# Murmeldyret/cubesat-APDS

Measured on AMD Instinct MI355X. Metric: frames/sec (detect+match+homography) 4k×4k tile vs 1M-desc DB; Mmatches/sec, higher is better.
Workload: dtype fp4 e2m1 operands / f32 accumulate = exact integer Hamming (match), f32 (AKAZE), f64 (homography solve)

## Files before the change

### cubesat-apds_amd/csrc/hamming_mfma.hip

```cpp
#include <atomic>
#include <memory>

#include "config.h"
#include "kernels.h"

namespace apds {

typedef int hm_v8i __attribute__((ext_vector_type(8)));
typedef float hm_f32x4 __attribute__((ext_vector_type(4)));
typedef uint32_t hm_u32x4 __attribute__((ext_vector_type(4)));

#ifndef APDS_HM_WAVES
#define APDS_HM_WAVES 8
#endif
static constexpr int HM_WAVES = APDS_HM_WAVES;
static constexpr int HM_TM = 16 * HM_WAVES;
#ifndef APDS_HM_WPE
#define APDS_HM_WPE 4
#endif
#ifndef APDS_HM_NC
#define APDS_HM_NC 3
#endif
static constexpr int HM_NC = APDS_HM_NC;
static constexpr int HM_Q = HM_WAVES * 16 * HM_NC;
static constexpr int HM_UNIT_SCALE = 0x7F7F7F7F;
static constexpr uint64_t HM_EMPTY = ~0ull;
static constexpr int HM_BIAS = 1024;

__device__ __forceinline__ uint32_t hm_spread8(uint32_t b, uint32_t nib) {
    uint32_t t = b & 0xFFu;
    t = (t | (t << 12)) & 0x000F000Fu;
    t = (t | (t << 6)) & 0x03030303u;
    t = (t | (t << 3)) & 0x11111111u;
    return t * nib;
}

__global__ __launch_bounds__(256) void hm_expand_rows_kernel(const uint32_t* __restrict__ rows, long long n, uint32_t nib, int bias, uint4* __restrict__ out,
                                                             float* __restrict__ pc) {
    APDS_RAISE_WAVE_PRIORITY();
    const long long i = (long long)blockIdx.x * 256 + threadIdx.x;
    const uint32_t d = i < n * 16 ? rows[i] : 0u;
    int v = __popc(d);
#pragma unroll
    for (int off = 8; off > 0; off >>= 1) v += __shfl_xor(v, off);
    if (i >= n * 16) return;
    out[i] = make_uint4(hm_spread8(d, nib), hm_spread8(d >> 8, nib), hm_spread8(d >> 16, nib), hm_spread8(d >> 24, nib));
    if ((threadIdx.x & 15) == 0) pc[i >> 4] = (float)(v + bias);
}

__global__ void hm_pad_rows_kernel(uint4* __restrict__ rows, float* __restrict__ pc, long long n, long long n_pad) {
    const long long i = n + (threadIdx.x >> 4);
    if (i >= n_pad) return;
    for (long long r = i; r < n_pad; r += 8) {
        rows[r * 16 + (threadIdx.x & 15)] = make_uint4(0, 0, 0, 0);
        if ((threadIdx.x & 15) == 0) pc[r] = INFINITY;
    }
}

__global__ void hm_thresholds_kernel(const uint64_t* __restrict__ topk, int K, const float* __restrict__ qpc, int nq, uint32_t* __restrict__ thr) {
    const int i = blockIdx.x * blockDim.x + threadIdx.x;
    if (i >= nq) return;
    const uint64_t k2 = topk[(size_t)i * K + K - 1];
    thr[i] = k2 == HM_EMPTY ? 0x7F800000u : __float_as_uint((float)((int)(uint32_t)(k2 >> 32) - (int)qpc[i] + HM_BIAS));
}

struct HmTop2 {
    uint32_t d0, d1;
    uint32_t i0, i1;
};
__device__ __forceinline__ void hm_insert(HmTop2& b, uint32_t d, uint32_t idx) {
    if (d < b.d1) {
        if (d < b.d0) {
            b.d1 = b.d0;
            b.i1 = b.i0;
            b.d0 = d;
            b.i0 = idx;
        } else {
            b.d1 = d;
            b.i1 = idx;
        }
    }
}

__device__ __forceinline__ void hm_dma_rows(const unsigned char* tile_base, const int (&voff)[4], uint32_t lds_dst) {
    uint32_t keep;
    asm volatile(
        "s_mov_b32 %0, m0\n\t"
        "s_mov_b32 m0, %6\n\t"
        "s_nop 0\n\t"
        "global_load_lds_dwordx4 %1, %5\n\t"
        "global_load_lds_dwordx4 %2, %5 offset:1024\n\t"
        "global_load_lds_dwordx4 %3, %5 offset:2048\n\t"
        "global_load_lds_dwordx4 %4, %5 offset:3072\n\t"
        "s_mov_b32 m0, %0"
        : "=&s"(keep)
        : "v"(voff[0]), "v"(voff[1]), "v"(voff[2]), "v"(voff[3]), "s"(tile_base), "s"(lds_dst)
        : "memory");
}
__device__ __forceinline__ void hm_dma_popcounts(const float* src, int voff, uint32_t lds_dst) {
    uint32_t keep;
    asm volatile(
        "s_mov_b32 %0, m0\n\t"
        "s_mov_b32 m0, %3\n\t"
        "s_nop 0\n\t"
        "global_load_lds_dword %1, %2\n\t"
        "s_mov_b32 m0, %0"
        : "=&s"(keep)
        : "v"(voff), "s"(src), "s"(lds_dst)
        : "memory");
}
__device__ __forceinline__ void hm_dma_wait() { asm volatile("s_waitcnt vmcnt(0)" ::: "memory"); }
template <class T>
__device__ __forceinline__ void hm_settle(T& v) { asm volatile("" : "+v"(v)); }

template <int NC, int PRIO, class Rank>
__device__ __forceinline__ void hm_scan_tiles(const uint4* __restrict__ train_fp4, const float* __restrict__ tpc, int tile_begin, int tile_end,
                                              uint4 (&B)[NC][4], uint32_t index_base, Rank&& rank) {
    extern __shared__ __attribute__((aligned(128))) unsigned char hm_lds[];
    constexpr int TILE_BYTES = HM_TM * 256;
    const int lane = threadIdx.x & 63, wave = __builtin_amdgcn_readfirstlane(threadIdx.x >> 6);
    const int col = lane & 15, kq = lane >> 4;
    const uint32_t lds0 = (uint32_t)(__SIZE_TYPE__)(__attribute__((address_space(3))) unsigned char*)hm_lds;
    int voff[4];
#pragma unroll
    for (int i = 0; i < 4; i++) {
        const int r = 16 * wave + 4 * i + (lane >> 4);
        voff[i] = r * 256 + (((lane & 15) ^ (r & 15)) << 4) - 1024 * i;
    }
    auto stage = [&](int tile, int buf) {
        hm_dma_rows(reinterpret_cast<const unsigned char*>(train_fp4) + (size_t)tile * TILE_BYTES, voff, lds0 + buf * TILE_BYTES + 16 * wave * 256);
        if (wave < HM_TM / 64) hm_dma_popcounts(tpc + (size_t)tile * HM_TM + 64 * wave, 4 * lane, lds0 + 2 * TILE_BYTES + buf * (HM_TM * 4) + 256 * wave);
    };
    typedef const __attribute__((address_space(3))) hm_u32x4* lds_u4;
    typedef const __attribute__((address_space(3))) hm_f32x4* lds_f4;
    uint32_t ra[4], rn = lds0 + 2 * TILE_BYTES + 16 * kq;
#pragma unroll
    for (int s = 0; s < 4; s++) ra[s] = lds0 + col * 256 + (((4 * s + kq) ^ col) << 4);

    hm_u32x4 a[4];
    hm_f32x4 init;
    auto read_block = [&](int rb) {
#pragma unroll
        for (int s = 0; s < 4; s++) a[s] = *(lds_u4)(__SIZE_TYPE__)(ra[s] + rb * 4096);
        init = *(lds_f4)(__SIZE_TYPE__)(rn + rb * 64);
    };

#pragma unroll
    for (int c = 0; c < NC; c++)
#pragma unroll
        for (int s = 0; s < 4; s++) hm_settle(B[c][s].x), hm_settle(B[c][s].y), hm_settle(B[c][s].z), hm_settle(B[c][s].w);
    hm_dma_wait();
    stage(tile_begin, 0);
    hm_dma_wait();
    __syncthreads();
    read_block(0);
    hm_f32x4 acc[NC];
    for (int tile = tile_begin; tile < tile_end; tile++) {
        const int buf = (tile - tile_begin) & 1;
        if (tile + 1 < tile_end) stage(tile + 1, buf ^ 1);
#pragma unroll
        for (int rb = 0; rb < HM_TM / 16; rb++) {
            if (PRIO) __builtin_amdgcn_s_setprio(PRIO);
#pragma unroll
            for (int s = 0; s < 4; s++) {
                const hm_v8i A = {(int)a[s].x, (int)a[s].y, (int)a[s].z, (int)a[s].w, 0, 0, 0, 0};
#pragma unroll
                for (int c = 0; c < NC; c++) {
                    const hm_v8i Bv = {(int)B[c][s].x, (int)B[c][s].y, (int)B[c][s].z, (int)B[c][s].w, 0, 0, 0, 0};
                    acc[c] = __builtin_amdgcn_mfma_scale_f32_16x16x128_f8f6f4(A, Bv, s == 0 ? init : acc[c], 4, 4, 0, HM_UNIT_SCALE, 0, HM_UNIT_SCALE);
                }
            }
            if (PRIO) __builtin_amdgcn_s_setprio(0);
            if (rb + 1 < HM_TM / 16) {
                read_block(rb + 1);
            } else {
                hm_dma_wait();
                __syncthreads();
#pragma unroll
                for (int s = 0; s < 4; s++) ra[s] += buf ? -TILE_BYTES : TILE_BYTES;
                rn += buf ? -HM_TM * 4 : HM_TM * 4;
                read_block(0);
            }
#pragma unroll
            for (int c = 0; c < NC; c++) hm_settle(acc[c]);
            __builtin_amdgcn_sched_barrier(0);
            rank(acc, (uint32_t)(tile * HM_TM + rb * 16 + 4 * kq) + index_base);
        }
    }
}

template <int PRIO, bool THR>
__global__ __launch_bounds__(64 * HM_WAVES) __attribute__((amdgpu_waves_per_eu(APDS_HM_WPE, APDS_HM_WPE))) void hamming_mfma_kernel(const uint4* __restrict__ train_fp4, const float* __restrict__ tpc, int n_train,
                                                           const uint4* __restrict__ query_fp4, const float* __restrict__ qpc, int nq, int tiles_per_split,
                                                           int q_tiles, int splits, uint32_t index_base, const uint32_t* __restrict__ thr,
                                                           uint64_t* __restrict__ out) {
    const int tid = threadIdx.x, lane = tid & 63, wave = tid >> 6;
    int split, qtile;
    if ((splits & 7) == 0) {
        const int xcd = blockIdx.x & 7, j = blockIdx.x >> 3;
        split = xcd + 8 * (j / q_tiles);
        qtile = j % q_tiles;
    } else {
        split = blockIdx.x / q_tiles;
        qtile = blockIdx.x % q_tiles;
    }
    const int q0 = qtile * HM_Q + wave * 16 * HM_NC;
    const int n_tiles = (n_train + HM_TM - 1) / HM_TM;
    const int tile_begin = split * tiles_per_split, tile_end = min(n_tiles, tile_begin + tiles_per_split);
    const int col = lane & 15, kq = lane >> 4;

    uint4 B[HM_NC][4];
    float qq[HM_NC];
#pragma unroll
    for (int c = 0; c < HM_NC; c++) {
        const int qi = min(q0 + 16 * c + col, nq - 1);
#pragma unroll
        for (int s = 0; s < 4; s++) B[c][s] = query_fp4[(size_t)qi * 16 + 4 * s + kq];
        qq[c] = qpc[qi];
    }
    HmTop2 best[HM_NC];
#pragma unroll
    for (int c = 0; c < HM_NC; c++) {
        best[c].d0 = THR ? thr[min(q0 + 16 * c + col, nq - 1)] : 0x7F800000u;
        hm_settle(best[c].d0), hm_settle(qq[c]);
        best[c].d1 = best[c].d0;
        best[c].i0 = best[c].i1 = 0xFFFFFFFFu;
    }

    if (tile_begin < tile_end) {
        hm_scan_tiles<HM_NC, PRIO>(train_fp4, tpc, tile_begin, tile_end, B, index_base, [&](const hm_f32x4 (&a)[HM_NC], uint32_t row0) {
            bool hit[HM_NC];
#pragma unroll
            for (int c = 0; c < HM_NC; c++) {
                const uint32_t mn = min(min(__float_as_uint(a[c][0]), __float_as_uint(a[c][1])), min(__float_as_uint(a[c][2]), __float_as_uint(a[c][3])));
                hit[c] = mn < best[c].d1;
            }
#pragma unroll
            for (int c = 0; c < HM_NC; c++)
                if (__any(hit[c])) {
#pragma unroll
                    for (int j = 0; j < 4; j++) hm_insert(best[c], __float_as_uint(a[c][j]), row0 + j);
                }
        });
    }
#pragma unroll
    for (int c = 0; c < HM_NC; c++) {
        HmTop2 b = best[c];
#pragma unroll
        for (int off = 16; off < 64; off <<= 1) {
            const uint32_t od0 = (uint32_t)__shfl_xor((int)b.d0, off), od1 = (uint32_t)__shfl_xor((int)b.d1, off);
            const uint32_t oi0 = (uint32_t)__shfl_xor((int)b.i0, off), oi1 = (uint32_t)__shfl_xor((int)b.i1, off);
            HmTop2 m = b;
            auto ins = [&](uint32_t d, uint32_t i) {
                if (i == 0xFFFFFFFFu) return;
                if (d < m.d0 || (d == m.d0 && i < m.i0)) {
                    m.d1 = m.d0;
                    m.i1 = m.i0;
                    m.d0 = d;
                    m.i0 = i;
                } else if ((d < m.d1 || (d == m.d1 && i < m.i1)) && i != m.i0) {
                    m.d1 = d;
                    m.i1 = i;
                }
            };
            ins(od0, oi0);
            ins(od1, oi1);
            b = m;
        }
        const int qi = q0 + 16 * c + col;
        if (kq == 0 && qi < nq) {
            uint64_t* o = out + ((size_t)split * nq + qi) * 2;
            o[0] = b.i0 == 0xFFFFFFFFu ? HM_EMPTY : ((uint64_t)(uint32_t)((int)(qq[c] + __uint_as_float(b.d0)) - HM_BIAS) << 32) | b.i0;
            o[1] = b.i1 == 0xFFFFFFFFu ? HM_EMPTY : ((uint64_t)(uint32_t)((int)(qq[c] + __uint_as_float(b.d1)) - HM_BIAS) << 32) | b.i1;
        }
    }
}

template <int K>
struct HmTopK {
    uint32_t d[K];
    uint32_t i[K];
};
template <int K>
__device__ __forceinline__ void hm_insert_k(HmTopK<K>& b, uint32_t d, uint32_t idx) {
#pragma unroll
    for (int j = K - 1; j > 0; j--) {
        const bool shift = d < b.d[j - 1], here = d < b.d[j];
        b.i[j] = shift ? b.i[j - 1] : (here ? idx : b.i[j]);
        b.d[j] = shift ? b.d[j - 1] : (here ? d : b.d[j]);
    }
    const bool first = d < b.d[0];
    b.i[0] = first ? idx : b.i[0];
    b.d[0] = first ? d : b.d[0];
}
__device__ __forceinline__ uint64_t hm_shfl_xor_u64(uint64_t v, int off) {
    return ((uint64_t)(uint32_t)__shfl_xor((int)(uint32_t)(v >> 32), off) << 32) | (uint32_t)__shfl_xor((int)(uint32_t)v, off);
}

#ifndef APDS_HM_NC_K4
#define APDS_HM_NC_K4 2
#endif
#ifndef APDS_HM_NC_K8
#define APDS_HM_NC_K8 2
#endif
template <int K>
struct HmShape {
    static constexpr int NC = K <= 4 ? APDS_HM_NC_K4 : APDS_HM_NC_K8;
    static constexpr int Q = HM_WAVES * 16 * NC;
};

template <int K, int NC, int PRIO, bool THR>
__global__ __launch_bounds__(64 * HM_WAVES) __attribute__((amdgpu_waves_per_eu(APDS_HM_WPE, APDS_HM_WPE))) void hamming_mfma_topk_kernel(
    const uint4* __restrict__ train_fp4, const float* __restrict__ tpc, int n_train, const uint4* __restrict__ query_fp4, const float* __restrict__ qpc, int nq,
    int tiles_per_split, int q_tiles, int splits, uint32_t index_base, const uint32_t* __restrict__ thr, uint64_t* __restrict__ out) {
    const int tid = threadIdx.x, lane = tid & 63, wave = tid >> 6;
    int split, qtile;
    if ((splits & 7) == 0) {
        const int xcd = blockIdx.x & 7, j = blockIdx.x >> 3;
        split = xcd + 8 * (j / q_tiles);
        qtile = j % q_tiles;
    } else {
        split = blockIdx.x / q_tiles;
        qtile = blockIdx.x % q_tiles;
    }
    const int q0 = qtile * (HM_WAVES * 16 * NC) + wave * 16 * NC;
    const int n_tiles = (n_train + HM_TM - 1) / HM_TM;
    const int tile_begin = split * tiles_per_split, tile_end = min(n_tiles, tile_begin + tiles_per_split);
    const int col = lane & 15, kq = lane >> 4;

    uint4 B[NC][4];
    float qq[NC];
#pragma unroll
    for (int c = 0; c < NC; c++) {
        const int qi = min(q0 + 16 * c + col, nq - 1);
#pragma unroll
        for (int s = 0; s < 4; s++) B[c][s] = query_fp4[(size_t)qi * 16 + 4 * s + kq];
        qq[c] = qpc[qi];
    }
    HmTopK<K> best[NC];
#pragma unroll
    for (int c = 0; c < NC; c++) {
        uint32_t start = THR ? thr[min(q0 + 16 * c + col, nq - 1)] : 0x7F800000u;
        hm_settle(start), hm_settle(qq[c]);
#pragma unroll
        for (int j = 0; j < K; j++) best[c].d[j] = start, best[c].i[j] = 0xFFFFFFFFu;
    }

    if (tile_begin < tile_end) {
        hm_scan_tiles<NC, PRIO>(train_fp4, tpc, tile_begin, tile_end, B, index_base, [&](const hm_f32x4 (&a)[NC], uint32_t row0) {
            bool hit[NC];
#pragma unroll
            for (int c = 0; c < NC; c++) {
                const uint32_t mn = min(min(__float_as_uint(a[c][0]), __float_as_uint(a[c][1])), min(__float_as_uint(a[c][2]), __float_as_uint(a[c][3])));
                hit[c] = mn < best[c].d[K - 1];
            }
#pragma unroll
            for (int c = 0; c < NC; c++)
                if (__any(hit[c])) {
#pragma unroll
                    for (int j = 0; j < 4; j++) {
                        const uint32_t v = __float_as_uint(a[c][j]);
                        if (__any(v < best[c].d[K - 1])) hm_insert_k<K>(best[c], v, row0 + j);
                    }
                }
        });
    }
#pragma unroll
    for (int c = 0; c < NC; c++) {
        uint64_t key[K];
#pragma unroll
        for (int j = 0; j < K; j++) key[j] = ((uint64_t)best[c].d[j] << 32) | best[c].i[j];
#pragma unroll
        for (int off = 16; off < 64; off <<= 1) {
            uint64_t other[K];
#pragma unroll
            for (int j = 0; j < K; j++) other[j] = hm_shfl_xor_u64(key[j], off);
#pragma unroll
            for (int j = 0; j < K; j++) key[j] = min(key[j], other[K - 1 - j]);
#pragma unroll
            for (int step = K / 2; step > 0; step >>= 1)
#pragma unroll
                for (int j = 0; j < K; j++)
                    if ((j & step) == 0) {
                        const uint64_t lo = min(key[j], key[j + step]), hi = max(key[j], key[j + step]);
                        key[j] = lo;
                        key[j + step] = hi;
                    }
        }
        const int qi = q0 + 16 * c + col;
        if (kq == 0 && qi < nq) {
            uint64_t* o = out + ((size_t)split * nq + qi) * K;
#pragma unroll
            for (int j = 0; j < K; j++) {
                const uint32_t d = (uint32_t)(key[j] >> 32), i = (uint32_t)key[j];
                o[j] = i == 0xFFFFFFFFu ? HM_EMPTY : ((uint64_t)(uint32_t)((int)(qq[c] + __uint_as_float(d)) - HM_BIAS) << 32) | i;
            }
        }
    }
}

static int hm_list_len(int k) { return k <= 2 ? 2 : (k <= 4 ? 4 : 8); }
static int hm_queries_per_block(int K) { return K <= 2 ? HM_Q : (K <= 4 ? HmShape<4>::Q : HmShape<8>::Q); }

HmPlan hm_plan(int nq, long long nt, int K) {
    HmPlan p;
    p.q_tiles = ceil_div(nq, hm_queries_per_block(K));
    const int t_tiles = (int)ceil_div(nt, (long long)HM_TM);
    constexpr int SLOTS = 256 * (16 / HM_WAVES);
    constexpr int OVERHEAD = 4;
    const int max_splits = (int)std::max<long long>(1, std::min<long long>(std::min(t_tiles, 128), (32ll << 20) / std::max(K, 2) / std::max(nq, 1)));
    long long best_cost = -1;
    p.splits = 1;
    for (int sp = 1; sp <= max_splits; sp++) {
        const long long rounds = ceil_div((long long)p.q_tiles * sp, (long long)SLOTS);
        const long long cost = rounds * (ceil_div(t_tiles, sp) + OVERHEAD);
        if (best_cost < 0 || cost < best_cost) best_cost = cost, p.splits = sp;
    }
    if (config().match_mfma_xcd && t_tiles >= 64) {
        long long best8 = -1;
        int sp8 = 0;
        for (int sp = 8; sp <= std::min(max_splits, 32); sp += 8) {
            const long long rounds = ceil_div((long long)p.q_tiles * sp, (long long)SLOTS);
            const long long cost = rounds * (ceil_div(t_tiles, sp) + OVERHEAD);
            if (best8 < 0 || cost < best8) best8 = cost, sp8 = sp;
        }
        if (sp8 && best8 * 100 <= best_cost * 105) {
            p.splits = sp8;
            p.tiles_per_split = ceil_div(t_tiles, p.splits);
            return p;
        }
    }
    if (config().match_mfma_splits > 0) p.splits = std::min(t_tiles, config().match_mfma_splits);
    p.tiles_per_split = ceil_div(t_tiles, p.splits);
    p.splits = ceil_div(t_tiles, p.tiles_per_split);
    return p;
}

void hm_expand_device(const void* rows64, long long n, bool query, void* out_fp4, float* pc, hipStream_t s) {
    if (n <= 0) return;
    hipLaunchKernelGGL(hm_expand_rows_kernel, dim3((unsigned)ceil_div(n * 16, 256)), dim3(256), 0, s, static_cast<const uint32_t*>(rows64), n, query ? 0xCu : 0x2u,
                       query ? 0 : HM_BIAS, static_cast<uint4*>(out_fp4), pc);
    if (!query && hm_padded_rows(n) > n)
        hipLaunchKernelGGL(hm_pad_rows_kernel, dim3(1), dim3(128), 0, s, static_cast<uint4*>(out_fp4), pc, n, hm_padded_rows(n));
}
long long hm_padded_rows(long long n) { return ceil_div(n, (long long)HM_TM) * HM_TM; }
long long hm_sample_rows(long long nt) {
    const long long cap = config().match_mfma_sample;
    return (cap > 0 && nt >= 65536) ? std::min<long long>(cap, nt / 16 / HM_TM * HM_TM) / HM_TM * HM_TM : 0;
}

template <int K>
static void hm_scan_k_launch(const void* q_fp4, const float* qpc, int nq, const void* t_fp4, const float* tpc, long long nt, const HmPlan& p, uint32_t index_base,
                             uint64_t* parts, hipStream_t s, const uint32_t* thr, size_t lds) {
    constexpr int NC = HmShape<K>::NC;
    static std::atomic<bool> opted_dev[64];
    std::atomic<bool>& opted = opted_dev[ctx().device & 63];
    if (!opted.load()) {
        auto opt = [&](auto kernel) { HIP_CHECK(hipFuncSetAttribute(reinterpret_cast<const void*>(kernel), hipFuncAttributeMaxDynamicSharedMemorySize, 160 * 1024)); };
        opt(&hamming_mfma_topk_kernel<K, NC, 0, false>), opt(&hamming_mfma_topk_kernel<K, NC, 2, false>);
        opt(&hamming_mfma_topk_kernel<K, NC, 0, true>), opt(&hamming_mfma_topk_kernel<K, NC, 2, true>);
        opted.store(true);
    }
    auto go = [&](auto kernel) {
        hipLaunchKernelGGL(kernel, dim3((unsigned)p.q_tiles * p.splits), dim3(64 * HM_WAVES), lds, s, static_cast<const uint4*>(t_fp4), tpc, (int)nt,
                           static_cast<const uint4*>(q_fp4), qpc, nq, p.tiles_per_split, p.q_tiles, p.splits, index_base, thr, parts);
    };
    const bool prio = config().match_mfma_prio > 0;
    if (thr) prio ? go(&hamming_mfma_topk_kernel<K, NC, 2, true>) : go(&hamming_mfma_topk_kernel<K, NC, 0, true>);
    else prio ? go(&hamming_mfma_topk_kernel<K, NC, 2, false>) : go(&hamming_mfma_topk_kernel<K, NC, 0, false>);
}

void hm_scan_device(const void* q_fp4, const float* qpc, int nq, const void* t_fp4, const float* tpc, long long nt, const HmPlan& p, uint32_t index_base,
                    uint64_t* parts, hipStream_t s, const uint32_t* thr, bool timed, int K) {
    const size_t lds = (size_t)2 * HM_TM * 256 + 2 * HM_TM * sizeof(float) + (size_t)std::max(0, config().match_mfma_lds_pad);
    if (K > 2) {
        APDS_REQUIRE(K == 4 || K == 8, APDS_ERR_ASSERT, "the matrix-core matcher keeps lists of 2, 4 or 8");
        std::unique_ptr<KernelTimer> timer, timer_k;
        if (timed) timer.reset(new KernelTimer("hamming_topk", s)), timer_k.reset(new KernelTimer("hamming_topk_mfma_k", s));
        if (K == 4) hm_scan_k_launch<4>(q_fp4, qpc, nq, t_fp4, tpc, nt, p, index_base, parts, s, thr, lds);
        else hm_scan_k_launch<8>(q_fp4, qpc, nq, t_fp4, tpc, nt, p, index_base, parts, s, thr, lds);
        return;
    }
    static std::atomic<bool> opted_dev[64];
    std::atomic<bool>& opted = opted_dev[ctx().device & 63];
    if (!opted.load()) {
        auto opt = [&](auto kernel) { HIP_CHECK(hipFuncSetAttribute(reinterpret_cast<const void*>(kernel), hipFuncAttributeMaxDynamicSharedMemorySize, 160 * 1024)); };
        opt(&hamming_mfma_kernel<0, false>), opt(&hamming_mfma_kernel<1, false>), opt(&hamming_mfma_kernel<2, false>), opt(&hamming_mfma_kernel<3, false>);
        opt(&hamming_mfma_kernel<0, true>), opt(&hamming_mfma_kernel<1, true>), opt(&hamming_mfma_kernel<2, true>), opt(&hamming_mfma_kernel<3, true>);
        opted.store(true);
    }
    std::unique_ptr<KernelTimer> timer;
    if (timed) timer.reset(new KernelTimer("hamming_topk", s));
    auto go = [&](auto kernel) {
        hipLaunchKernelGGL(kernel, dim3((unsigned)p.q_tiles * p.splits), dim3(64 * HM_WAVES), lds, s, static_cast<const uint4*>(t_fp4), tpc, (int)nt,
                           static_cast<const uint4*>(q_fp4), qpc, nq, p.tiles_per_split, p.q_tiles, p.splits, index_base, thr, parts);
    };
    const int prio = std::max(0, std::min(3, config().match_mfma_prio));
    if (thr) {
        switch (prio) {
            case 0: go(&hamming_mfma_kernel<0, true>); break;
            case 1: go(&hamming_mfma_kernel<1, true>); break;
            case 2: go(&hamming_mfma_kernel<2, true>); break;
            default: go(&hamming_mfma_kernel<3, true>); break;
        }
    } else {
        switch (prio) {
            case 0: go(&hamming_mfma_kernel<0, false>); break;
            case 1: go(&hamming_mfma_kernel<1, false>); break;
            case 2: go(&hamming_mfma_kernel<2, false>); break;
            default: go(&hamming_mfma_kernel<3, false>); break;
        }
    }
}

void* hm_train_create(const void* rows64, long long n, hipStream_t s) {
    APDS_REQUIRE(rows64 && n > 0 && n < (1ll << 31), APDS_ERR_ASSERT, "an expanded train set needs rows");
    HmTrain* t = new HmTrain();
    t->device = ctx().device;
    t->src = rows64;
    t->n = n;
    if (hipMalloc(&t->rows, (size_t)hm_padded_rows(n) * 256) != hipSuccess || hipMalloc(reinterpret_cast<void**>(&t->pc), (size_t)hm_padded_rows(n) * 4) != hipSuccess) {
        (void)hipGetLastError();
        if (t->rows) (void)hipFree(t->rows);
        delete t;
        fail(APDS_ERR_NOMEM, "no device memory for the expanded train rows");
    }
    hm_expand_device(rows64, n, false, t->rows, t->pc, s);
    HIP_CHECK(hipStreamSynchronize(s));
    return t;
}
void hm_train_destroy(void* h) {
    HmTrain* t = static_cast<HmTrain*>(h);
    if (!t) return;
    int previous = -1;
    if (hipGetDevice(&previous) != hipSuccess) previous = -1;
    (void)hipSetDevice(t->device);
    (void)hipDeviceSynchronize();
    if (t->rows) (void)hipFree(t->rows);
    if (t->pc) (void)hipFree(t->pc);
    delete t;
    if (previous >= 0) (void)hipSetDevice(previous);
}

static void hm_topk_expanded(const void* q, int nq, const void* t4, const float* tp, long long nt, uint32_t index_base, int k, uint64_t* out, hipStream_t s) {
    ThreadCtx& c = ctx();
    void* q4 = c.alloc((size_t)nq * 256);
    float* qp = c.alloc_n<float>(nq);
    {
        KernelTimer timer("hamming_topk_sample", s);
        hm_expand_device(q, nq, true, q4, qp, s);
    }
    const long long sample = hm_sample_rows(nt);
    const int K = hm_list_len(k);
    uint64_t* topk = k == K ? out : c.alloc_n<uint64_t>((size_t)nq * K);
    if (sample) {
        const HmPlan pa = hm_plan(nq, sample, K), pb = hm_plan(nq, nt - sample, K);
        uint64_t* parts_a = c.alloc_n<uint64_t>((size_t)pa.splits * nq * K);
        uint64_t* parts_b = c.alloc_n<uint64_t>((size_t)(pb.splits + 1) * nq * K);
        uint64_t* topk_a = parts_b + (size_t)pb.splits * nq * K;
        uint32_t* thr = c.alloc_n<uint32_t>(nq);
        {
            KernelTimer timer("hamming_topk_sample", s);
            hm_scan_device(q4, qp, nq, t4, tp, sample, pa, index_base, parts_a, s, nullptr, false, K);
            if (pa.splits > 1) merge_topk_device(parts_a, pa.splits, nq, K, topk_a, s);
            else HIP_CHECK(hipMemcpyAsync(topk_a, parts_a, (size_t)nq * K * 8, hipMemcpyDeviceToDevice, s));
            hipLaunchKernelGGL(hm_thresholds_kernel, dim3(ceil_div(nq, 256)), dim3(256), 0, s, (const uint64_t*)topk_a, K, (const float*)qp, nq, thr);
        }
        hm_scan_device(q4, qp, nq, static_cast<const char*>(t4) + (size_t)sample * 256, tp + sample, nt - sample, pb, index_base + (uint32_t)sample, parts_b, s, thr,
                       true, K);
        merge_topk_device(parts_b, pb.splits + 1, nq, K, topk, s);
    } else {
        const HmPlan p = hm_plan(nq, nt, K);
        uint64_t* parts = p.splits == 1 ? topk : c.alloc_n<uint64_t>((size_t)p.splits * nq * K);
        hm_scan_device(q4, qp, nq, t4, tp, nt, p, index_base, parts, s, nullptr, true, K);
        if (p.splits > 1) merge_topk_device(parts, p.splits, nq, K, topk, s);
    }
    if (k != K) take_first_columns_device(topk, nq, K, k, out, s);
    HIP_CHECK(hipGetLastError());
}

void hamming_mfma_topk_device(const void* q, int nq, const void* t, long long nt, uint32_t index_base, int k, uint64_t* out, hipStream_t s) {
    APDS_REQUIRE(k >= 1 && k <= 8, APDS_ERR_ASSERT, "the matrix-core matcher serves 1 <= k <= 8");
    APDS_REQUIRE(nq > 0 && nt > 0 && nt < (1ll << 31), APDS_ERR_ASSERT, "the matrix-core matcher needs queries and train rows");
    ThreadCtx& c = ctx();
    void* t4 = c.alloc((size_t)hm_padded_rows(nt) * 256);
    float* tp = c.alloc_n<float>(hm_padded_rows(nt));
    {
        KernelTimer timer("hamming_topk_sample", s);
        hm_expand_device(t, nt, false, t4, tp, s);
    }
    hm_topk_expanded(q, nq, t4, tp, nt, index_base, k, out, s);
}

void hamming_mfma_topk_train_device(const void* q, int nq, const void* train, uint32_t index_base, int k, uint64_t* out, hipStream_t s) {
    const HmTrain* t = static_cast<const HmTrain*>(train);
    APDS_REQUIRE(t && k >= 1 && k <= 8 && nq > 0, APDS_ERR_ASSERT, "the matrix-core matcher needs an expanded train set, queries and 1 <= k <= 8");
    hm_topk_expanded(q, nq, t->rows, t->pc, t->n, index_base, k, out, s);
}

}
```

Baseline: 149.7.

## Software-pipeline MFMA Hamming scan with inline asm interleaving previous block's rank test

Replaces the compiler-scheduled MFMA loop with hand-written inline-asm blocks. The min/compare filter for the previous row block is interleaved between the MFMAs of the current one, using two ping-pong accumulator sets, and a drain step handles the final block. The aim is to hide the rank-test VALU work and the MFMA result latency behind matrix-core issue instead of serialising them. It also defers the query popcount load to the epilogue to free registers. This adds fragile asm with hard-coded operand modifiers and an s_nop hazard, supports only NC of 2 or 3, and increases live accumulator registers.

```diff
diff --git a/cubesat-apds_amd/csrc/hamming_mfma.hip b/cubesat-apds_amd/csrc/hamming_mfma.hip
--- a/cubesat-apds_amd/csrc/hamming_mfma.hip
+++ b/cubesat-apds_amd/csrc/hamming_mfma.hip
@@ -113,11 +113,74 @@
 template <class T>
 __device__ __forceinline__ void hm_settle(T& v) { asm volatile("" : "+v"(v)); }
 
-template <int NC, int PRIO, class Rank>
+#define HM_MFMA(D, BQ, C) "v_mfma_scale_f32_16x16x128_f8f6f4 " D ", %[a], " BQ ", " C ", %[sc], %[sc] op_sel_hi:[0,0,0] cbsz:4 blgp:4\n\t"
+#define HM_MIN3 "v_min3_u32 %[t], %[y0], %[y1], %[y2]\n\t"
+#define HM_MIN "v_min_u32 %[t], %[t], %[y3]\n\t"
+#define HM_CMP "v_cmp_lt_u32_e64 %[hit], %[t], %[bd]\n\t"
+#define HM_RANK_OPERANDS(y, bound) [y0] "v"(y[0]), [y1] "v"(y[1]), [y2] "v"(y[2]), [y3] "v"(y[3]), [bd] "v"(bound)
+
+template <int S>
+__device__ __forceinline__ void hm_step3(hm_f32x4 (&x)[3], const hm_u32x4& a, const hm_u32x4 (&B)[3][4], const hm_f32x4& init, int scale, const hm_f32x4& y,
+                                         uint32_t bound, uint64_t& hit) {
+    uint32_t t;
+    if constexpr (S == 0)
+        asm volatile(HM_MFMA("%[x0]", "%[b0]", "%[c]") HM_MFMA("%[x1]", "%[b1]", "%[c]") HM_MIN3 HM_MFMA("%[x2]", "%[b2]", "%[c]") HM_MIN HM_CMP
+                     : [x0] "=&v"(x[0]), [x1] "=&v"(x[1]), [x2] "=&v"(x[2]), [t] "=&v"(t), [hit] "=&s"(hit)
+                     : [a] "v"(a), [b0] "v"(B[0][0]), [b1] "v"(B[1][0]), [b2] "v"(B[2][0]), [c] "v"(init), [sc] "v"(scale), HM_RANK_OPERANDS(y, bound));
+    else if constexpr (S < 3)
+        asm volatile(HM_MFMA("%[x0]", "%[b0]", "%[x0]") HM_MFMA("%[x1]", "%[b1]", "%[x1]") HM_MIN3 HM_MFMA("%[x2]", "%[b2]", "%[x2]") HM_MIN HM_CMP
+                     : [x0] "+v"(x[0]), [x1] "+v"(x[1]), [x2] "+v"(x[2]), [t] "=&v"(t), [hit] "=&s"(hit)
+                     : [a] "v"(a), [b0] "v"(B[0][S]), [b1] "v"(B[1][S]), [b2] "v"(B[2][S]), [sc] "v"(scale), HM_RANK_OPERANDS(y, bound));
+    else
+        asm volatile(HM_MFMA("%[x0]", "%[b0]", "%[x0]") HM_MFMA("%[x1]", "%[b1]", "%[x1]") HM_MFMA("%[x2]", "%[b2]", "%[x2]")
+                     : [x0] "+v"(x[0]), [x1] "+v"(x[1]), [x2] "+v"(x[2])
+                     : [a] "v"(a), [b0] "v"(B[0][S]), [b1] "v"(B[1][S]), [b2] "v"(B[2][S]), [sc] "v"(scale));
+}
+template <int S>
+__device__ __forceinline__ void hm_step2(hm_f32x4 (&x)[2], const hm_u32x4& a, const hm_u32x4 (&B)[2][4], const hm_f32x4& init, int scale, const hm_f32x4& y,
+                                         uint32_t bound, uint64_t& hit) {
+    uint32_t t;
+    if constexpr (S == 0)
+        asm volatile(HM_MFMA("%[x0]", "%[b0]", "%[c]") HM_MFMA("%[x1]", "%[b1]", "%[c]")
+                     : [x0] "=&v"(x[0]), [x1] "=&v"(x[1])
+                     : [a] "v"(a), [b0] "v"(B[0][0]), [b1] "v"(B[1][0]), [c] "v"(init), [sc] "v"(scale));
+    else if constexpr (S < 3)
+        asm volatile(HM_MFMA("%[x0]", "%[b0]", "%[x0]") HM_MFMA("%[x1]", "%[b1]", "%[x1]") HM_MIN3 HM_MIN HM_CMP
+                     : [x0] "+v"(x[0]), [x1] "+v"(x[1]), [t] "=&v"(t), [hit] "=&s"(hit)
+                     : [a] "v"(a), [b0] "v"(B[0][S]), [b1] "v"(B[1][S]), [sc] "v"(scale), HM_RANK_OPERANDS(y, bound));
+    else
+        asm volatile(HM_MFMA("%[x0]", "%[b0]", "%[x0]") HM_MFMA("%[x1]", "%[b1]", "%[x1]")
+                     : [x0] "+v"(x[0]), [x1] "+v"(x[1])
+                     : [a] "v"(a), [b0] "v"(B[0][S]), [b1] "v"(B[1][S]), [sc] "v"(scale));
+}
+template <int NC, class Bound>
+__device__ __forceinline__ void hm_block(hm_f32x4 (&x)[NC], const hm_f32x4 (&y)[NC], const hm_u32x4 (&a)[4], const hm_u32x4 (&B)[NC][4], const hm_f32x4& init,
+                                         int scale, Bound&& bound, uint64_t (&hit)[NC]) {
+    static_assert(NC == 2 || NC == 3, "a block body is written for two and for three column blocks");
+    if constexpr (NC == 3) {
+        hm_step3<0>(x, a[0], B, init, scale, y[0], bound(0), hit[0]);
+        hm_step3<1>(x, a[1], B, init, scale, y[1], bound(1), hit[1]);
+        hm_step3<2>(x, a[2], B, init, scale, y[2], bound(2), hit[2]);
+        hm_step3<3>(x, a[3], B, init, scale, y[0], 0u, hit[0]);
+    } else {
+        hm_step2<0>(x, a[0], B, init, scale, y[0], 0u, hit[0]);
+        hm_step2<1>(x, a[1], B, init, scale, y[0], bound(0), hit[0]);
+        hm_step2<2>(x, a[2], B, init, scale, y[1], bound(1), hit[1]);
+        hm_step2<3>(x, a[3], B, init, scale, y[0], 0u, hit[0]);
+    }
+}
+#undef HM_MFMA
+#undef HM_MIN3
+#undef HM_MIN
+#undef HM_CMP
+#undef HM_RANK_OPERANDS
+
+template <int NC, int PRIO, class Bound, class Insert>
 __device__ __forceinline__ void hm_scan_tiles(const uint4* __restrict__ train_fp4, const float* __restrict__ tpc, int tile_begin, int tile_end,
-                                              uint4 (&B)[NC][4], uint32_t index_base, Rank&& rank) {
+                                              uint4 (&Bq)[NC][4], uint32_t index_base, Bound&& bound, Insert&& insert) {
     extern __shared__ __attribute__((aligned(128))) unsigned char hm_lds[];
     constexpr int TILE_BYTES = HM_TM * 256;
+    static_assert(HM_TM / 16 % 2 == 0, "the two accumulator sets change roles an even number of times per tile");
     const int lane = threadIdx.x & 63, wave = __builtin_amdgcn_readfirstlane(threadIdx.x >> 6);
     const int col = lane & 15, kq = lane >> 4;
     const uint32_t lds0 = (uint32_t)(__SIZE_TYPE__)(__attribute__((address_space(3))) unsigned char*)hm_lds;
@@ -144,32 +207,43 @@
         for (int s = 0; s < 4; s++) a[s] = *(lds_u4)(__SIZE_TYPE__)(ra[s] + rb * 4096);
         init = *(lds_f4)(__SIZE_TYPE__)(rn + rb * 64);
     };
+    auto insert_hits = [&](const uint64_t (&hit)[NC], const hm_f32x4 (&v)[NC], uint32_t row0) {
+        uint64_t any = hit[0];
+#pragma unroll
+        for (int c = 1; c < NC; c++) any |= hit[c];
+        if (any) {
+#pragma unroll
+            for (int c = 0; c < NC; c++)
+                if (hit[c]) insert(c, v[c], row0);
+        }
+    };
 
 #pragma unroll
     for (int c = 0; c < NC; c++)
 #pragma unroll
-        for (int s = 0; s < 4; s++) hm_settle(B[c][s].x), hm_settle(B[c][s].y), hm_settle(B[c][s].z), hm_settle(B[c][s].w);
+        for (int s = 0; s < 4; s++) hm_settle(Bq[c][s].x), hm_settle(Bq[c][s].y), hm_settle(Bq[c][s].z), hm_settle(Bq[c][s].w);
+    hm_u32x4 B[NC][4];
+#pragma unroll
+    for (int c = 0; c < NC; c++)
+#pragma unroll
+        for (int s = 0; s < 4; s++) B[c][s] = hm_u32x4{Bq[c][s].x, Bq[c][s].y, Bq[c][s].z, Bq[c][s].w};
+    int scale = HM_UNIT_SCALE;
+    hm_settle(scale);
     hm_dma_wait();
     stage(tile_begin, 0);
     hm_dma_wait();
     __syncthreads();
     read_block(0);
-    hm_f32x4 acc[NC];
+    hm_f32x4 even[NC], odd[NC];
+#pragma unroll
+    for (int c = 0; c < NC; c++) odd[c] = hm_f32x4{INFINITY, INFINITY, INFINITY, INFINITY};
     for (int tile = tile_begin; tile < tile_end; tile++) {
         const int buf = (tile - tile_begin) & 1;
         if (tile + 1 < tile_end) stage(tile + 1, buf ^ 1);
-#pragma unroll
-        for (int rb = 0; rb < HM_TM / 16; rb++) {
+        auto block = [&](hm_f32x4 (&x)[NC], hm_f32x4 (&y)[NC], int rb) {
+            uint64_t hit[NC];
             if (PRIO) __builtin_amdgcn_s_setprio(PRIO);
-#pragma unroll
-            for (int s = 0; s < 4; s++) {
-                const hm_v8i A = {(int)a[s].x, (int)a[s].y, (int)a[s].z, (int)a[s].w, 0, 0, 0, 0};
-#pragma unroll
-                for (int c = 0; c < NC; c++) {
-                    const hm_v8i Bv = {(int)B[c][s].x, (int)B[c][s].y, (int)B[c][s].z, (int)B[c][s].w, 0, 0, 0, 0};
-                    acc[c] = __builtin_amdgcn_mfma_scale_f32_16x16x128_f8f6f4(A, Bv, s == 0 ? init : acc[c], 4, 4, 0, HM_UNIT_SCALE, 0, HM_UNIT_SCALE);
-                }
-            }
+            hm_block<NC>(x, y, a, B, init, scale, bound, hit);
             if (PRIO) __builtin_amdgcn_s_setprio(0);
             if (rb + 1 < HM_TM / 16) {
                 read_block(rb + 1);
@@ -181,12 +255,23 @@
                 rn += buf ? -HM_TM * 4 : HM_TM * 4;
                 read_block(0);
             }
-#pragma unroll
-            for (int c = 0; c < NC; c++) hm_settle(acc[c]);
-            __builtin_amdgcn_sched_barrier(0);
-            rank(acc, (uint32_t)(tile * HM_TM + rb * 16 + 4 * kq) + index_base);
-        }
-    }
+            insert_hits(hit, y, (uint32_t)(tile * HM_TM + (rb - 1) * 16 + 4 * kq) + index_base);
+        };
+#pragma unroll
+        for (int rb = 0; rb < HM_TM / 16; rb += 2) {
+            block(even, odd, rb);
+            block(odd, even, rb + 1);
+        }
+    }
+#pragma unroll
+    for (int c = 0; c < NC; c++) asm volatile("s_nop 5" : "+v"(odd[c]));
+    uint64_t hit[NC];
+#pragma unroll
+    for (int c = 0; c < NC; c++) {
+        const uint32_t mn = min(min(__float_as_uint(odd[c][0]), __float_as_uint(odd[c][1])), min(__float_as_uint(odd[c][2]), __float_as_uint(odd[c][3])));
+        hit[c] = __ballot(mn < bound(c));
+    }
+    insert_hits(hit, odd, (uint32_t)(tile_end * HM_TM - 16 + 4 * kq) + index_base);
 }
 
 template <int PRIO, bool THR>
@@ -210,38 +295,28 @@
     const int col = lane & 15, kq = lane >> 4;
 
     uint4 B[HM_NC][4];
-    float qq[HM_NC];
 #pragma unroll
     for (int c = 0; c < HM_NC; c++) {
         const int qi = min(q0 + 16 * c + col, nq - 1);
 #pragma unroll
         for (int s = 0; s < 4; s++) B[c][s] = query_fp4[(size_t)qi * 16 + 4 * s + kq];
-        qq[c] = qpc[qi];
     }
     HmTop2 best[HM_NC];
 #pragma unroll
     for (int c = 0; c < HM_NC; c++) {
         best[c].d0 = THR ? thr[min(q0 + 16 * c + col, nq - 1)] : 0x7F800000u;
-        hm_settle(best[c].d0), hm_settle(qq[c]);
+        hm_settle(best[c].d0);
         best[c].d1 = best[c].d0;
         best[c].i0 = best[c].i1 = 0xFFFFFFFFu;
     }
 
     if (tile_begin < tile_end) {
-        hm_scan_tiles<HM_NC, PRIO>(train_fp4, tpc, tile_begin, tile_end, B, index_base, [&](const hm_f32x4 (&a)[HM_NC], uint32_t row0) {
-            bool hit[HM_NC];
-#pragma unroll
-            for (int c = 0; c < HM_NC; c++) {
-                const uint32_t mn = min(min(__float_as_uint(a[c][0]), __float_as_uint(a[c][1])), min(__float_as_uint(a[c][2]), __float_as_uint(a[c][3])));
-                hit[c] = mn < best[c].d1;
-            }
-#pragma unroll
-            for (int c = 0; c < HM_NC; c++)
-                if (__any(hit[c])) {
-#pragma unroll
-                    for (int j = 0; j < 4; j++) hm_insert(best[c], __float_as_uint(a[c][j]), row0 + j);
-                }
-        });
+        hm_scan_tiles<HM_NC, PRIO>(
+            train_fp4, tpc, tile_begin, tile_end, B, index_base, [&](int c) { return best[c].d1; },
+            [&](int c, const hm_f32x4& v, uint32_t row0) {
+#pragma unroll
+                for (int j = 0; j < 4; j++) hm_insert(best[c], __float_as_uint(v[j]), row0 + j);
+            });
     }
 #pragma unroll
     for (int c = 0; c < HM_NC; c++) {
@@ -269,9 +344,10 @@
         }
         const int qi = q0 + 16 * c + col;
         if (kq == 0 && qi < nq) {
+            const float qq = qpc[qi];
             uint64_t* o = out + ((size_t)split * nq + qi) * 2;
-            o[0] = b.i0 == 0xFFFFFFFFu ? HM_EMPTY : ((uint64_t)(uint32_t)((int)(qq[c] + __uint_as_float(b.d0)) - HM_BIAS) << 32) | b.i0;
-            o[1] = b.i1 == 0xFFFFFFFFu ? HM_EMPTY : ((uint64_t)(uint32_t)((int)(qq[c] + __uint_as_float(b.d1)) - HM_BIAS) << 32) | b.i1;
+            o[0] = b.i0 == 0xFFFFFFFFu ? HM_EMPTY : ((uint64_t)(uint32_t)((int)(qq + __uint_as_float(b.d0)) - HM_BIAS) << 32) | b.i0;
+            o[1] = b.i1 == 0xFFFFFFFFu ? HM_EMPTY : ((uint64_t)(uint32_t)((int)(qq + __uint_as_float(b.d1)) - HM_BIAS) << 32) | b.i1;
         }
     }
 }
@@ -347,23 +423,15 @@
     }
 
     if (tile_begin < tile_end) {
-        hm_scan_tiles<NC, PRIO>(train_fp4, tpc, tile_begin, tile_end, B, index_base, [&](const hm_f32x4 (&a)[NC], uint32_t row0) {
-            bool hit[NC];
-#pragma unroll
-            for (int c = 0; c < NC; c++) {
-                const uint32_t mn = min(min(__float_as_uint(a[c][0]), __float_as_uint(a[c][1])), min(__float_as_uint(a[c][2]), __float_as_uint(a[c][3])));
-                hit[c] = mn < best[c].d[K - 1];
-            }
-#pragma unroll
-            for (int c = 0; c < NC; c++)
-                if (__any(hit[c])) {
-#pragma unroll
-                    for (int j = 0; j < 4; j++) {
-                        const uint32_t v = __float_as_uint(a[c][j]);
-                        if (__any(v < best[c].d[K - 1])) hm_insert_k<K>(best[c], v, row0 + j);
-                    }
+        hm_scan_tiles<NC, PRIO>(
+            train_fp4, tpc, tile_begin, tile_end, B, index_base, [&](int c) { return best[c].d[K - 1]; },
+            [&](int c, const hm_f32x4& v, uint32_t row0) {
+#pragma unroll
+                for (int j = 0; j < 4; j++) {
+                    const uint32_t d = __float_as_uint(v[j]);
+                    if (__any(d < best[c].d[K - 1])) hm_insert_k<K>(best[c], d, row0 + j);
                 }
-        });
+            });
     }
 #pragma unroll
     for (int c = 0; c < NC; c++) {
```

After: 148.9. No clear change (-0.5%).
